# payakorn/InteriorPointMethod

Hardware: AMD Instinct MI355X
Metric: IPM iterations/sec (m=4096,n=8192 dense LP) (higher is better)
Workload: dtype f64; 1 GPU; dense synthetic LP m=4096 n=8192 fp64, seed 0, start x=s=1 y=0 (BASELINE.json configs[1]); replicas per GPU

## Files before the change

interiorpointmethod_amd/csrc/host_factor_solve.h:

```cpp
#pragma once
static inline bool sp_on(const ipm_handle* h) { return h->spf && !h->spf_off; }
static inline bool sp_level(const ipm_handle* h) {
    if (h->sp_serial || h->sp_level_mode < 0) return false;
    if (h->sp_level_mode > 0 || (h->opt.flags & IPM_FLAG_NO_DEVICE_POLLING)) return true;
    return !alone_on_device(h);
}
static inline unsigned sp_launch_grid(ipm_handle* h) {
    if (h->sp_serial) { ++h->sp_serial_launches; return 1u; }
    return (unsigned)h->sp_grid;
}
template <class Launch>
static void sp_walk(ipm_handle* h, bool by_level, bool leaves_first, Launch launch) {
    if (!by_level) { launch(sp_launch_grid(h), h->spF.rec, 0); return; }
    const size_t nlev = h->sp_lvlptr.empty() ? 0 : h->sp_lvlptr.size() - 1;
    for (size_t i = 0; i < nlev; ++i) {
        const size_t l = leaves_first ? i : nlev - 1 - i;
        const int cnt = h->sp_lvlptr[l + 1] - h->sp_lvlptr[l];
        launch((unsigned)std::min(cnt, h->sp_grid), h->sp_rec_level + h->sp_lvlptr[l], cnt);
    }
}

static int ensure_dense_B(ipm_handle* h) {
    if (h->B && h->invD) return IPM_OK;
    if (!h->no_dense) return fail(h, IPM_ERR_STATE, "handle has no dense normal-matrix buffer");
// ... 238 lines not shown
    a.L = h->B; a.ld = h->mp; a.inv = h->invD; a.done = &h->sc->done;
    a.r = r; a.z = z; a.j0 = 0;
    for (int k = k0; k < h->nblk; ++k) {
        a.k = k;
        const int nb = h->use_env ? h->env_last[k] - k + 1 : h->nblk - k;
        launch_twin<LS_TRSV_FWD>(h, (unsigned)nb, a);
    }
    a.r = z; a.z = out;
    for (int k = h->nblk - 1; k >= k0; --k) {
        a.k = k;
        a.j0 = h->use_env ? h->env_first[k] : 0;
        launch_twin<LS_TRSV_BWD>(h, (unsigned)(k - a.j0 + 1), a);
    }
}

static int enqueue_potrs_grouped(ipm_handle* h, double* r, double* out, hipEvent_t wait_last = nullptr) {
    const int GS = h->gsz;
    const int GR = GS * 128;
    const int nG = h->nblk / GS;
    const int* done = &h->sc->done;
    double* z = h->t2;
    for (int g = 0; g < nG; ++g) {
        if (wait_last && g == nG - 1) HIP_TRY(h, hipStreamWaitEvent(h->stream, wait_last, 0));
        launch_dense_gemv_n(h, h->gX + (int64_t)g * GR * GR, GR, GR, GR, r + (int64_t)g * GR, 1.0, 0.0, nullptr, z + (int64_t)g * GR);
        int below = (int)(h->mp - (int64_t)(g + 1) * GR);
        if (h->use_env) below = std::min(below, (int)((int64_t)(h->env_last[(g + 1) * GS - 1] + 1) * NB - (int64_t)(g + 1) * GR));
        if (below > 0) {
            double* rb = r + (int64_t)(g + 1) * GR;
            launch_dense_gemv_n(h, h->B + (int64_t)(g + 1) * GR * h->mp + (int64_t)g * GR, h->mp, below, GR, z + (int64_t)g * GR, -1.0, 1.0,
                                rb, rb);
        }
    }
    enqueue_block_steps(h, nG * GS, r, z, out);
    for (int g = nG - 1; g >= 0; --g) {
        launch_dense_gemv_n(h, h->gXT + (int64_t)g * GR * GR, GR, GR, GR, z + (int64_t)g * GR, 1.0, 0.0, nullptr, out + (int64_t)g * GR);
        int left = g * GR;
        const int c0 = h->use_env ? std::min(left, h->env_first[g * GS] * NB) : 0;
        left -= c0;
        if (left > 0) {
            const unsigned gx = (unsigned)((left + 511) / 512);
            launch_twin<LS_GEMV_T>(h, gx * 16u, {h->B + (int64_t)g * GR * h->mp + c0, h->mp, GR / 16, left, out + (int64_t)g * GR, h->gPart, done, gx});
            launch_twin<LS_SUB_PARTIALS>(h, (unsigned)((left + 255) / 256), {z + c0, h->gPart, left, 16, done});
        }
    }
    HIP_TRY(h, hipGetLastError());
    return IPM_OK;
}

static int enqueue_potrs(ipm_handle* h, double* r, double* out, hipEvent_t wait_last = nullptr) {
    if (sp_on(h)) {
        const int rm = std::max(16, h->sp_rmax);
        unsigned ep = ++h->sp_epoch;
        const bool fwd_done = h->sp_fwd_fused != nullptr && h->sp_fwd_fused == r;
        h->sp_fwd_fused = nullptr;
        const bool by_level = sp_level(h);
        if (!fwd_done) sp_walk(h, by_level, true, [&](unsigned grid, const SpRec* recs, int count) {
            hipLaunchKernelGGL((sp_fwd_kernel<SPC_THREADS, false>), dim3(grid), dim3(SPC_THREADS), h->sp_lds_solve, h->stream, h->spF, ep, r, h->t2, rm, recs, count);
        });
        if (!by_level) ep = ++h->sp_epoch;
        sp_walk(h, by_level, false, [&](unsigned grid, const SpRec* recs, int count) {
            hipLaunchKernelGGL((sp_bwd_kernel<SPC_THREADS, false>), dim3(grid), dim3(SPC_THREADS), 0, h->stream, h->spF, ep, h->t2, out, recs, count);
        });
        HIP_TRY(h, hipGetLastError());
        return IPM_OK;
    }
    if (h->grouped_trsv) return enqueue_potrs_grouped(h, r, out, wait_last);
    if (wait_last) HIP_TRY(h, hipStreamWaitEvent(h->stream, wait_last, 0));
    enqueue_block_steps(h, 0, r, h->t2, out);
    HIP_TRY(h, hipGetLastError());
    return IPM_OK;
}
```

interiorpointmethod_amd/csrc/host_fused.h:

```cpp
#pragma once
static bool ff_ok(const ipm_handle* h) {
    if (!h->ff_enabled || h->sparse || !polls_device(h)) return false;
    if (h->nblk < h->ff_min_nblk || h->nblk > std::min(h->ff_max_nblk, FF_MAX_NBLK) || h->np % FF_PBK) return false;
    return h->ff_forced || h->np <= 6 * h->mp;
}

static int ff_build(ipm_handle* h) {
    if (h->ff_built) return IPM_OK;
    {
        hipDeviceProp_t prop;
        HIP_TRY(h, hipGetDeviceProperties(&prop, h->device));
        if (!h->ff_forced && (strncmp(prop.gcnArchName, "gfx950", 6) != 0 || prop.multiProcessorCount != 256))
            return fail(h, IPM_ERR_STATE, "fused factor: built for a 256-CU gfx950 device (this one: %s, %d CUs)", prop.gcnArchName, prop.multiProcessorCount);
    }
    if (h->ff_workers <= 0) {
        hipDeviceProp_t prop;
        HIP_TRY(h, hipGetDeviceProperties(&prop, h->device));
        h->ff_workers = std::max(8, prop.multiProcessorCount - 1 - FF_CRIT_WGS);
    }
    const int nstages = (int)(h->np / FF_PBK);
    const int Q = std::max(1, std::min(h->ff_q, nstages));
    h->ff_q = Q;
    FFModel M;
    M.nstages = nstages;
// ... 20 lines not shown
        for (int i = 0; i < h->nblk; ++i)
            for (int c = 0; c <= i; ++c) {
                const size_t t = (size_t)ff_tile(i, c);
                if (fcnt[t] != h->ff_sched.tile_q[t] || base[t] != 1 || applied[t] != ff_limit(i, c) || paneled[t] != (ff_needs_panel(i, c) ? 1 : 0))
                    return fail(h, IPM_ERR_INVALID_ARG, "fused factor: internal error (tile %d,%d incomplete in the work list)", i, c);
            }
    }
    const size_t nit = h->ff_sched.items.size();
    HIP_TRY(h, dev_malloc(h->device, h->stream, (void**)&h->d_ff_items, sizeof(FFItem) * nit));
    HIP_TRY(h, hipMemcpyAsync(h->d_ff_items, h->ff_sched.items.data(), sizeof(FFItem) * nit, hipMemcpyHostToDevice, h->stream));
    HIP_TRY(h, dev_malloc(h->device, h->stream, (void**)&h->d_ff_tile_items, sizeof(int) * 2 * ntile));
    HIP_TRY(h, hipMemcpyAsync(h->d_ff_tile_items, h->ff_sched.tile_items.data(), sizeof(int) * ntile, hipMemcpyHostToDevice, h->stream));
    HIP_TRY(h, hipMemcpyAsync(h->d_ff_tile_items + ntile, h->ff_sched.tile_q.data(), sizeof(int) * ntile, hipMemcpyHostToDevice, h->stream));
    h->ff_flag_words = 32 + 2 * ntile + 3 * (size_t)h->nblk;
    HIP_TRY(h, dev_malloc(h->device, h->stream, (void**)&h->d_ff_flags, sizeof(unsigned) * 2 * h->ff_flag_words));
    HIP_TRY(h, dev_malloc(h->device, h->stream, (void**)&h->ff_slab, sizeof(double) * ntile * (size_t)h->ff_qmax * 128 * 128));
    if (getenv("IPM_FF_PROF")) {
        HIP_TRY(h, dev_malloc(h->device, h->stream, (void**)&h->ff_prof, sizeof(long long) * 16 * ((size_t)h->ff_workers + 1)));
        HIP_TRY(h, hipMemsetAsync(h->ff_prof, 0, sizeof(long long) * 16 * ((size_t)h->ff_workers + 1), h->stream));
    }
    if (getenv("IPM_FF_TRACE_ITEMS")) {
        const size_t words = 4 * nit + 12 * (size_t)h->nblk;
        HIP_TRY(h, dev_malloc(h->device, h->stream, (void**)&h->ff_trace, sizeof(long long) * words));
        HIP_TRY(h, hipMemsetAsync(h->ff_trace, 0, sizeof(long long) * words, h->stream));
    }
    HIP_TRY(h, hipStreamSynchronize(h->stream));
    h->ff_built = true;
    return IPM_OK;
}

static void ff_release(ipm_handle* h) {
    for (void** p : {(void**)&h->d_ff_items, (void**)&h->d_ff_flags, (void**)&h->ff_slab, (void**)&h->ff_prof, (void**)&h->ff_trace,
                     (void**)&h->d_ff_tile_items}) { dev_free(h->device, h->stream, *p); *p = nullptr; }
    h->ff_built = false;
}
static bool ff_use(ipm_handle* h) {
    if (!ff_ok(h)) return false;
    if (h->ff_built) return true;
    if (ff_build(h) == IPM_OK) return true;
    ff_release(h);
    h->ff_enabled = 0;
    (void)hipGetLastError();
    return false;
}

static int enqueue_form_factor(ipm_handle* h, hipEvent_t* ev, int mid_step, int ginv_step) {
    if (!h->ff_built) return fail(h, IPM_ERR_STATE, "fused factor: schedule not built");
    const int nblk = h->nblk;
    const size_t ntile = (size_t)nblk * (nblk + 1) / 2;
    const int* done = factor_done(h);
    hipStream_t sw = h->stream;
    unsigned* F = h->d_ff_flags;
    unsigned *ticket = F, *dbg = F + 24, *fcount = F + 32, *tprog = fcount + ntile, *lfinal = tprog + ntile, *dready = lfinal + nblk,
             *potrfdone = dready + nblk;
    unsigned* timeout = timeout_word(h);
    h->ff_potrfdone = potrfdone;
    HIP_TRY(h, hipMemsetAsync(F, 0, sizeof(unsigned) * h->ff_flag_words, sw));
    HIP_TRY(h, hipEventRecord(h->ev_fork, sw));
    long long* ctrace = h->ff_trace ? h->ff_trace + 4 * h->ff_sched.items.size() : nullptr;
    FFRoles roles;
    memset(&roles, 0, sizeof roles);
    FFChain& c = roles.chain;
    c.B = h->B; c.ldb = h->mp; c.invD = h->invD;
    c.maxbits = (const unsigned long long*)(F + 8); c.dcount = F + 10; c.maxdiag_out = &h->sc->maxdiag;
    c.dready = dready; c.potrfdone = potrfdone; c.timeout = timeout; c.dbg = dbg; c.trace = ctrace;
    c.eps = h->opt.pivot_guard_eps; c.big = h->opt.pivot_guard_big; c.shift_rel = h->shift_rel;
    c.fixed = &h->sc->fixed; c.done = done; c.nblk = nblk; c.m = (int)h->m;
    FFCrit& cc = roles.crit;
    cc.B = h->B; cc.ldb = h->mp; cc.invD = h->invD; cc.tprog = tprog; cc.tile_items = h->d_ff_tile_items;
    cc.potrfdone = potrfdone; cc.lfinal = lfinal; cc.dready = dready; cc.timeout = timeout; cc.dbg = dbg; cc.trace = ctrace;
    cc.done = done; cc.nblk = nblk;
    roles.role = F + 3;
    FFArgs a;
    memset(&a, 0, sizeof a);
    a.A = h->A; a.lda = h->np; a.d = h->d; a.B = h->B; a.ldb = h->mp; a.invD = h->invD; a.slab = h->ff_slab;
    a.items = h->d_ff_items; a.nitems = (int)h->ff_sched.items.size();
    a.ticket = ticket; a.fcount = fcount; a.tprog = tprog; a.lfinal = lfinal; a.dready = dready; a.potrfdone = potrfdone;
    a.timeout = timeout; a.dbg = dbg; a.done = done;
    { static const bool dbg_on = getenv("IPM_FF_DEBUG") != nullptr; a.dbg_words = dbg_on ? (unsigned)h->ff_flag_words : 0u; }
    a.trace = h->ff_trace;
    a.prof = h->ff_prof;
    a.tile_q = h->d_ff_tile_items + ntile;
    a.maxbits = (unsigned long long*)(F + 8); a.dcount = F + 10;
    a.nblk = nblk; a.Q = h->ff_qmax; a.nstages = (int)(h->np / FF_PBK); a.m = (int)h->m;
    if (ev) HIP_TRY(h, hipEventRecord(ev[1], sw));
    {
        const dim3 grid((unsigned)h->ff_workers + 1u + (unsigned)FF_CRIT_WGS);
        const bool instr = a.prof || a.trace;
        if (h->ff_ref_engine) {
            if (instr) hipLaunchKernelGGL((form_factor_roles_kernel<true>), grid, dim3(FF_THREADS), 0, sw, a, roles);
// ... 113 lines not shown
```

interiorpointmethod_amd/csrc/host_handle.h:

```cpp
#pragma once
static thread_local char g_err[512] = "";

static const int MAX_DEVICES = 64;
static std::atomic<int> g_live[MAX_DEVICES];
static std::atomic<bool> g_attr_set[MAX_DEVICES];

struct ipm_handle {
    int device = 0;
    hipStream_t stream = nullptr;
    bool own_stream = false;
    hipStream_t stream2 = nullptr;
    hipStream_t stream3 = nullptr;
    hipEvent_t ev_mid = nullptr, ev_res = nullptr, ev_grp = nullptr, ev_last = nullptr;
    std::vector<hipEvent_t> ev_crit, ev_bulk;
    hipEvent_t ev_fork = nullptr;
    int lookahead = 1;
    int grouped_trsv = 1;
    int gsz = 0;
    double *gXT = nullptr, *gX = nullptr, *gS = nullptr, *gPart = nullptr;
    unsigned* d_bulk_done = nullptr;
    bool no_dense = false;
    double* B_own = nullptr; double* invD_own = nullptr;
    int group_steps = 0;
    int two_level = 1;
// ... 65 lines not shown
    std::vector<int> env_last, env_first;
    bool use_env = false;
    int envelope = 1;
    bool sparse = false;
    int64_t nnz_cap = 0, nnz = 0;
    int* d_tile_order = nullptr;
    int *d_rowptr = nullptr, *d_colind = nullptr, *d_colptr = nullptr, *d_rowind = nullptr;
    double *d_rval = nullptr, *d_cval = nullptr;
    long long* stamp_buf = nullptr;
    unsigned* ff_potrfdone = nullptr;
    Scalars* sc = nullptr;
    IterRec* hist = nullptr;
    double* snap = nullptr;
    bool bnd = false;
    int bnd_nU = 0;
    double* bnd_mem = nullptr;
    bool detect = false;
    double det_eps_p = 1e-8, det_eps_d = 1e-8;
    double* det = nullptr;
    double* cert_mem = nullptr;
    int* fixed = nullptr;
    Scalars* h_sc = nullptr;
    bool haveA = false, haveBC = false, haveState = false, predictor_valid = false;
    bool fresh_state = true;
    int profiling = 0;
    double phase_ms[4] = {0, 0, 0, 0};
    hipEvent_t ev0 = nullptr, ev1 = nullptr;
    std::vector<struct LsLaunch>* ls_rec = nullptr;
    bool ls_cut = false;
    int lockstep = 0;
    unsigned spin_limit = 1u << 22;
    bool ragged_groups = true;
    bool ls_block_steps = false, potrf_stamps = false, ff_chain_mode0 = false;
    char err[512] = "";
};
struct LsLaunch { int type; LsRec rec; };
template <LsType T> static void record_twin(ipm_handle* h, unsigned gridx, const LsArgs<T>& a, unsigned lds = 0) {
    LsLaunch L{};
    L.type = T; L.rec.gridx = gridx; L.rec.lds = lds;
    memcpy(L.rec.args, &a, sizeof a);
    h->ls_rec->push_back(L);
}
template <LsType T> static void launch_twin(ipm_handle* h, unsigned grid, const LsArgs<T>& a, hipStream_t st = nullptr, unsigned lds = 0) {
    if (h->ls_rec) record_twin<T>(h, grid, a, lds);
    else LsTwin<T>::single(a, grid, lds, st ? st : h->stream);
}
template <class... P, class... Q> static void launch_untwinned(ipm_handle* h, void (*kernel)(P...), dim3 grid, dim3 block, hipStream_t st, const Q&... args) {
    if (h->ls_rec) h->ls_cut = true;
    else hipLaunchKernelGGL(kernel, grid, block, 0, st ? st : h->stream, args...);
}

static int vfail(char* err, int code, const char* fmt, va_list ap) {
    char buf[512];
    vsnprintf(buf, sizeof buf, fmt, ap);
    snprintf(g_err, sizeof g_err, "%s", buf);
    if (err) snprintf(err, 512, "%s", buf);
    return code;
}
static int fail(ipm_handle* h, int code, const char* fmt, ...) { va_list ap; va_start(ap, fmt); code = vfail(h ? h->err : nullptr, code, fmt, ap); va_end(ap); return code; }

#define HIP_TRY(h, call)                                                                      \
    do {                                                                                      \
        hipError_t e_ = (call);                                                               \
        if (e_ != hipSuccess)                                                                 \
            return fail((h), IPM_ERR_HIP, "%s failed: %s (%s:%d)", #call, hipGetErrorString(e_), \
                        __FILE__, __LINE__);                                                  \
    } while (0)

static inline int64_t round_up(int64_t v, int64_t q) { return (v + q - 1) / q * q; }

static inline int live_on_device(const ipm_handle* h) { return h->device < MAX_DEVICES ? g_live[h->device].load(std::memory_order_acquire) : 1; }
static inline bool alone_on_device(const ipm_handle* h) { return live_on_device(h) <= 1; }
static inline bool lookahead_on(const ipm_handle* h) { return h->lookahead != 0 && h->nblk > 2 && h->stream2 != nullptr; }
static inline bool wants_polling(const ipm_handle* h) { return lookahead_on(h) && h->flag_sync != 0; }
static inline bool polls_device(const ipm_handle* h) { return wants_polling(h) && alone_on_device(h); }
static inline unsigned* timeout_word(const ipm_handle* h) { return h->d_flags + 2 * (size_t)h->nblk; }
static inline const int* factor_done(const ipm_handle* h) { return h->fdone ? h->fdone : &h->sc->done; }

static std::atomic<int> g_pool_state[64];
static hipMemPool_t g_pool[64];
static std::mutex g_pool_mutex;
static bool async_alloc_ok(int device) {
    if (device < 0 || device >= 64) return false;
    int st = g_pool_state[device].load(std::memory_order_acquire);
    if (st == 0) {
        std::lock_guard<std::mutex> lock(g_pool_mutex);
        st = g_pool_state[device].load(std::memory_order_acquire);
        if (st != 0) return st == 1;
        int supported = 0;
        if (hipDeviceGetAttribute(&supported, hipDeviceAttributeMemoryPoolsSupported, device) == hipSuccess && supported) {
            hipMemPoolProps props;
            memset(&props, 0, sizeof props);
            props.allocType = hipMemAllocationTypePinned;
            props.handleTypes = hipMemHandleTypeNone;
            props.location.type = hipMemLocationTypeDevice;
            props.location.id = device;
            hipMemPool_t pool = nullptr;
            if (hipMemPoolCreate(&pool, &props) == hipSuccess && pool) {
                uint64_t keep = (uint64_t)2 << 30;
                (void)hipMemPoolSetAttribute(pool, hipMemPoolAttrReleaseThreshold, &keep);
                g_pool[device] = pool;
                st = 1;
            }
        }
        if (st == 0) st = 2;
        g_pool_state[device].store(st, std::memory_order_release);
    }
    return st == 1;
}
// ... 111 lines not shown
```

interiorpointmethod_amd/csrc/host_iteration.h:

```cpp
#pragma once
static int enqueue_solve_direction(ipm_handle* h, hipEvent_t* ev, double* dy, int corr, hipEvent_t wait_last = nullptr) {
    if (ev) HIP_TRY(h, hipEventRecord(ev[0], h->stream));
    int rc = enqueue_potrs(h, h->t1, dy, wait_last);
    if (rc) return rc;
    if (ev) HIP_TRY(h, hipEventRecord(ev[1], h->stream));
    launch_gemv_t(h, dy);
    launch_direction(h, corr);
    HIP_TRY(h, hipGetLastError());
    return IPM_OK;
}
static int enqueue_predictor(ipm_handle* h, hipEvent_t* ev, bool have_rhs = false, hipEvent_t wait_last = nullptr) {
    if (!have_rhs) launch_gemv_n(h, h->v, -1.0, -1.0, h->rb, h->t1);
    return enqueue_solve_direction(h, ev, h->dya, 0, wait_last);
}
static int enqueue_corrector(ipm_handle* h, hipEvent_t* ev) {
    launch_mu_aff(h);
    launch_corrector_rhs(h);
    launch_gemv_n(h, h->v, -1.0, -1.0, h->rb, h->t1);
    return enqueue_solve_direction(h, ev, h->dy, 1);
}

static const int EV_PER_IT = 9;

static int enqueue_iteration(ipm_handle* h, hipEvent_t* ev) {
    int rc;
    const bool all = ev && h->profiling >= 2;
    if (overlap_residuals(h)) {
        launch_scaling(h);
        const bool fused = ff_use(h);
        if (ev && !fused) HIP_TRY(h, hipEventRecord(ev[1], h->stream));
        struct Latch { ipm_handle* h; ~Latch() { h->fdone = nullptr; } } latch{h};
        h->fdone = &h->sc->done_f;
        h->ff_last = false;
        if (!fused) {
            if ((rc = enqueue_form(h, h->d))) return rc;
            if (ev) HIP_TRY(h, hipEventRecord(ev[2], h->stream));
        }
        const int rstep = h->nblk * 13 / 16;
        const int nG = h->grouped_trsv ? h->nblk / h->gsz : 0;
        const int gstep = (nG >= 2 && (nG - 1) * h->gsz - 1 < rstep) ? (nG - 1) * h->gsz - 1 : -1;
        if (fused) { if ((rc = enqueue_form_factor(h, ev, rstep, gstep))) return rc; }
        else if ((rc = enqueue_factor(h, true, rstep, gstep))) return rc;
        h->fdone = nullptr;
        if (gstep >= 0) {
            if (h->ff_last && h->ff_potrfdone) {
                hipLaunchKernelGGL(ff_gate_kernel, dim3(1), dim3(64), 0, h->stream3, h->ff_potrfdone + (h->nblk - 1), 1u, timeout_word(h), &h->sc->done);
            } else {
                HIP_TRY(h, hipEventRecord(h->ev_grp, h->stream));
                HIP_TRY(h, hipStreamWaitEvent(h->stream3, h->ev_grp, 0));
            }
            if ((rc = enqueue_group_inverses(h, nG - 1, nG, h->stream3))) return rc;
            HIP_TRY(h, hipEventRecord(h->ev_last, h->stream3));
            HIP_TRY(h, hipStreamWaitEvent(h->stream, h->ev_res, 0));
            if ((rc = enqueue_predictor(h, nullptr, true, h->ev_last))) return rc;
        } else {
            if ((rc = enqueue_group_inverses(h, 0, nG, nullptr))) return rc;
            HIP_TRY(h, hipStreamWaitEvent(h->stream, h->ev_res, 0));
            if ((rc = enqueue_predictor(h, nullptr, true))) return rc;
        }
        if ((rc = enqueue_corrector(h, nullptr))) return rc;
        launch_update(h);
        HIP_TRY(h, hipGetLastError());
        return IPM_OK;
    }
    if (all) HIP_TRY(h, hipEventRecord(ev[0], h->stream));
    if ((rc = enqueue_residuals(h))) return rc;
    h->ff_last = false;
    bool have_rhs = false;
    if (h->profiling < 2 && ff_use(h)) {
        if ((rc = enqueue_form_factor(h, ev, -1, -1))) return rc;
    } else {
        if (ev) HIP_TRY(h, hipEventRecord(ev[1], h->stream));
        if ((rc = enqueue_form(h, h->d))) return rc;
        if (ev) HIP_TRY(h, hipEventRecord(ev[2], h->stream));
        if (sp_on(h) && h->sp_fuse_fwd) {
            launch_gemv_n(h, h->v, -1.0, -1.0, h->rb, h->t1);
            have_rhs = true;
            if ((rc = enqueue_factor(h, true, -1, -1, h->t1))) return rc;
        } else if ((rc = enqueue_factor(h, true))) return rc;
    }
    if ((rc = enqueue_group_inverses(h))) return rc;
    if (all) HIP_TRY(h, hipEventRecord(ev[3], h->stream));
    if ((rc = enqueue_predictor(h, all ? ev + 4 : nullptr, have_rhs))) return rc;
    if ((rc = enqueue_corrector(h, all ? ev + 6 : nullptr))) return rc;
    launch_update(h);
    HIP_TRY(h, hipGetLastError());
    if (all) HIP_TRY(h, hipEventRecord(ev[8], h->stream));
    return IPM_OK;
}

static int read_scalars(ipm_handle* h, bool* timed_out = nullptr) {
    unsigned tmo = 0;
    unsigned* word = timeout_word(h);
    HIP_TRY(h, hipMemcpyAsync(h->h_sc, h->sc, sizeof(Scalars), hipMemcpyDeviceToHost, h->stream));
// ... 9 lines not shown
    return IPM_OK;
}

static void poll_fallback(ipm_handle* h) {
    if (h->spf) h->sp_serial = true;
    if (h->ff_last) h->ff_enabled = 0;
    else h->flag_sync = 0;
    ++h->timeouts_recovered;
}

__global__ __launch_bounds__(256) void snapshot_kernel(double* x, double* y, double* s, Scalars* sc, double* snap, int np,
                                                       int mp, int restore) {
    const int gid = blockIdx.x * 256 + threadIdx.x, gsz = gridDim.x * 256;
    double *sx = snap, *ss = snap + np, *sy = snap + 2 * (size_t)np;
    Scalars* ssc = (Scalars*)(snap + 2 * (size_t)np + mp);
    if (restore) {
        for (int j = gid; j < np; j += gsz) { x[j] = sx[j]; s[j] = ss[j]; }
        for (int i = gid; i < mp; i += gsz) y[i] = sy[i];
        if (gid == 0) *sc = *ssc;
    } else {
        for (int j = gid; j < np; j += gsz) { sx[j] = x[j]; ss[j] = s[j]; }
        for (int i = gid; i < mp; i += gsz) sy[i] = y[i];
        if (gid == 0) *ssc = *sc;
    }
}
__global__ __launch_bounds__(256) void snapshot_bounds_kernel(double* w, double* z, double* sw, double* sz, int np, int restore) {
    const int gid = blockIdx.x * 256 + threadIdx.x, gsz = gridDim.x * 256;
    for (int j = gid; j < np; j += gsz) {
        if (restore) { w[j] = sw[j]; z[j] = sz[j]; }
        else { sw[j] = w[j]; sz[j] = z[j]; }
    }
}
static int enqueue_snapshot(ipm_handle* h, int restore, hipStream_t st = nullptr) {
    const int64_t mx = h->np > h->mp ? h->np : h->mp;
    const unsigned grid = (unsigned)std::min<int64_t>((mx + 255) / 256, 256);
    hipLaunchKernelGGL(snapshot_kernel, dim3(grid), dim3(256), 0, st ? st : h->stream, h->x, h->y, h->s, h->sc, h->snap, (int)h->np,
                       (int)h->mp, restore);
    if (h->bnd) {
        const BndArgs b = bnd_args(h);
        double* sw = h->bnd_mem + 8 * (size_t)h->np;
        hipLaunchKernelGGL(snapshot_bounds_kernel, dim3(grid), dim3(256), 0, st ? st : h->stream, b.w, b.z, sw, sw + h->np, (int)h->np, restore);
    }
    HIP_TRY(h, hipGetLastError());
    return IPM_OK;
}
static bool may_poll(const ipm_handle* h) { return (h->spf && !h->sp_serial && !sp_level(h)) || wants_polling(h); }

static void fill_stats(ipm_handle* h, ipm_stats* st, double ms) {
    if (!st) return;
    const Scalars& s = *h->h_sc;
    memset(st, 0, sizeof *st);
    st->status = s.status; st->iterations = s.k; st->pivots_fixed = s.fixed; st->auto_regularized = h->auto_reg;
    st->objective_last_finite = s.obj_last_finite;
    st->objective = s.obj; st->rp_norm = s.rb_norm; st->rd_norm = s.rc_norm; st->gap = s.gap;
    st->b_norm = s.b_norm; st->c_norm = s.c_norm; st->mu = s.mu; st->mu_aff = s.mu_aff; st->sigma = s.sigma;
    st->alpha_aff_p = s.alpha_aff_p; st->alpha_aff_d = s.alpha_aff_d; st->alpha_p = s.alpha_p; st->alpha_d = s.alpha_d;
    st->solve_ms = ms;
}

static int check_ready(ipm_handle* h, const char* who) {
    if (!h) return fail(h, IPM_ERR_INVALID_ARG, "%s: NULL handle", who);
    if (!h->haveA || !h->haveBC || !h->haveState) return fail(h, IPM_ERR_STATE, "%s: A, (b,c) and a state must be set first", who);
    return IPM_OK;
}

extern "C" int ipm_newton_direction(ipm_handle* h, int corrector, double* dx, double* dy, double* ds, ipm_stats* stats) {
// ... 29 lines not shown
    if (corrector && (rc = read_scalars(h))) return rc;
    HIP_TRY(h, hipStreamSynchronize(h->stream));
    fill_stats(h, stats, 0.0);
    return IPM_OK;
}

static SmallLP small_args(ipm_handle* h, int max_steps, int auto_reg) {
    SmallLP a;
    a.A = sparse_view(h); a.m = (int)h->m; a.n = (int)h->n; a.nt = (int)((h->m + 15) / 16);
    a.bptr = h->sm_bptr; a.bi = h->sm_bi; a.bk = h->sm_bk; a.bcol = h->sm_bcol; a.bcoef = h->sm_bcoef; a.nb = h->sm_nb;
    a.x = h->x; a.y = h->y; a.s = h->s; a.b = h->b; a.c = h->c;
    a.rc = h->rc; a.d = h->d; a.v = h->v; a.q = h->q; a.dxa = h->dxa; a.dsa = h->dsa; a.dx = h->dx; a.ds = h->ds;
    a.sc = h->sc; a.hist = h->hist;
    a.eps = h->opt.pivot_guard_eps; a.big = h->opt.pivot_guard_big; a.shift_rel = h->shift_rel;
    a.max_steps = max_steps; a.auto_reg = auto_reg;
    return a;
}

static int enqueue_small(ipm_handle* h, int max_steps, int auto_reg) {
    const SmallLP a = small_args(h, max_steps, auto_reg);
    if (h->bnd && h->detect) hipLaunchKernelGGL(small_lp_bounded_detect_kernel, dim3(1), dim3(PD_THREADS), 0, h->stream, a, bnd_args(h), det_args(h));
    else if (h->bnd) hipLaunchKernelGGL(small_lp_bounded_kernel, dim3(1), dim3(PD_THREADS), 0, h->stream, a, bnd_args(h));
    else if (h->detect) hipLaunchKernelGGL(small_lp_detect_kernel, dim3(1), dim3(PD_THREADS), 0, h->stream, a, det_args(h));
    else hipLaunchKernelGGL(small_lp_kernel, dim3(1), dim3(PD_THREADS), 0, h->stream, a);
    HIP_TRY(h, hipGetLastError());
    return IPM_OK;
}

extern "C" int ipm_iterate(ipm_handle* h, int32_t n_steps, ipm_stats* stats) {
    int rc = check_ready(h, "ipm_iterate");
    if (rc) return rc;
    if (n_steps < 0) return fail(h, IPM_ERR_INVALID_ARG, "n_steps < 0");
    HIP_TRY(h, hipSetDevice(h->device));
    h->predictor_valid = false;
    std::vector<hipEvent_t> evs;
    struct EvGuard {
        std::vector<hipEvent_t>& v;
        ~EvGuard() { for (auto& e : v) if (e) (void)hipEventDestroy(e); }
    } guard{evs};
    if (h->profiling) {
        evs.assign((size_t)EV_PER_IT * n_steps, nullptr);
        for (auto& e : evs) HIP_TRY(h, hipEventCreate(&e));
    }
    float ms = 0.f;
    const int reset_k = h->fresh_state ? 1 : 0;
    h->fresh_state = false;
    if (h->small && !h->profiling) {
        hipLaunchKernelGGL(set_params_kernel, dim3(1), dim3(1), 0, h->stream, h->sc, 1e-8, 1e-8, 1e-8, h->opt.eta, 1 << 30, 1, reset_k);
        HIP_TRY(h, hipEventRecord(h->ev0, h->stream));
        if ((rc = enqueue_small(h, n_steps, 0))) return rc;
        HIP_TRY(h, hipEventRecord(h->ev1, h->stream));
        if ((rc = read_scalars(h))) return rc;
        HIP_TRY(h, hipEventElapsedTime(&ms, h->ev0, h->ev1));
        fill_stats(h, stats, ms);
        return IPM_OK;
    }
    for (int attempt = 0;; ++attempt) {
        hipLaunchKernelGGL(set_params_kernel, dim3(1), dim3(1), 0, h->stream, h->sc, 1e-8, 1e-8, 1e-8, h->opt.eta, 1 << 30, 1,
                           attempt == 0 ? reset_k : 0);
        const bool guard_poll = may_poll(h) && n_steps > 0;
        if (guard_poll && (rc = enqueue_snapshot(h, 0))) return rc;
        HIP_TRY(h, hipEventRecord(h->ev0, h->stream));
        for (int it = 0; it < n_steps; ++it)
            if ((rc = enqueue_iteration(h, h->profiling ? &evs[(size_t)it * EV_PER_IT] : nullptr))) return rc;
        if ((rc = enqueue_residuals(h))) return rc;
        HIP_TRY(h, hipEventRecord(h->ev1, h->stream));
        bool tmo = false;
        if ((rc = read_scalars(h, &tmo))) return rc;
        if (!tmo) break;
        if (attempt >= 2 || !guard_poll) return fail(h, IPM_ERR_HIP, "hand-off time-out persists with stream events");
        poll_fallback(h);
        if ((rc = enqueue_snapshot(h, 1))) return rc;
    }
    HIP_TRY(h, hipEventElapsedTime(&ms, h->ev0, h->ev1));
    if (h->profiling && n_steps > 0) {
        double ph[4] = {0, 0, 0, 0};
        for (int it = 0; it < n_steps; ++it) {
            hipEvent_t* e = &evs[(size_t)it * EV_PER_IT];
            float f = 0.f, total = 0.f;
            (void)hipEventElapsedTime(&f, e[1], e[2]); ph[0] += f;
            if (h->profiling < 2) continue;
            (void)hipEventElapsedTime(&f, e[2], e[3]); ph[1] += f;
            float s1 = 0.f, s2 = 0.f;
            (void)hipEventElapsedTime(&s1, e[4], e[5]); (void)hipEventElapsedTime(&s2, e[6], e[7]); ph[2] += s1 + s2;
            (void)hipEventElapsedTime(&total, e[0], e[8]);
            float f12 = 0.f, f23 = 0.f;
            (void)hipEventElapsedTime(&f12, e[1], e[2]); (void)hipEventElapsedTime(&f23, e[2], e[3]);
            ph[3] += total - f12 - f23 - s1 - s2;
        }
        for (int i = 0; i < 4; ++i) h->phase_ms[i] = ph[i] / n_steps;
    }
    fill_stats(h, stats, ms);
    return IPM_OK;
}

extern "C" int ipm_solve(ipm_handle* h, double tol_p, double tol_d, double tol_gap, int32_t max_iter, ipm_stats* stats) {
    int rc = check_ready(h, "ipm_solve");
    if (rc) return rc;
    if (max_iter < 0) return fail(h, IPM_ERR_INVALID_ARG, "max_iter < 0");
    HIP_TRY(h, hipSetDevice(h->device));
    h->predictor_valid = false; h->fresh_state = false;
    if (h->auto_reg) { h->auto_reg = 0; h->shift_rel = h->opt.regularize; }
    hipLaunchKernelGGL(set_params_kernel, dim3(1), dim3(1), 0, h->stream, h->sc, tol_p, tol_d, tol_gap, h->opt.eta, max_iter, 0, 1);
    HIP_TRY(h, hipEventRecord(h->ev0, h->stream));
    const int chunk = h->opt.check_every;
    const bool may_auto = h->opt.regularize == 0.0 && !(h->opt.flags & IPM_FLAG_NO_AUTO_REGULARIZE);
    if (h->small) {
        if ((rc = enqueue_small(h, 1 << 30, may_auto ? 1 : 0))) return rc;
        if ((rc = read_scalars(h))) return rc;
        if (h->h_sc->status == IPM_STATUS_NEEDS_SHIFT) {
            h->shift_rel = 1e-14; h->auto_reg = 1;
            hipLaunchKernelGGL(set_params_kernel, dim3(1), dim3(1), 0, h->stream, h->sc, tol_p, tol_d, tol_gap, h->opt.eta, max_iter, 0, 1);
            if ((rc = enqueue_small(h, 1 << 30, 0))) return rc;
            if ((rc = read_scalars(h))) return rc;
        }
        HIP_TRY(h, hipEventRecord(h->ev1, h->stream));
        HIP_TRY(h, hipEventSynchronize(h->ev1));
        float ms_ = 0.f;
        HIP_TRY(h, hipEventElapsedTime(&ms_, h->ev0, h->ev1));
        fill_stats(h, stats, ms_);
        return IPM_OK;
    }
    bool first = true;
    int recovered = 0;
    for (;;) {
        const bool snap = first || may_poll(h);
        if (snap && (rc = enqueue_snapshot(h, 0))) return rc;
        for (int i = 0; i < chunk; ++i)
            if ((rc = enqueue_iteration(h, nullptr))) return rc;
        bool tmo = false;
        if ((rc = read_scalars(h, &tmo))) return rc;
        if (tmo) {
            if (!snap || ++recovered > 2) return fail(h, IPM_ERR_HIP, "hand-off time-out persists with stream events");
            poll_fallback(h);
// ... 20 lines not shown
```

interiorpointmethod_amd/csrc/host_residuals.h:

```cpp
#pragma once
static void launch_gemv_n(ipm_handle* h, const double* v, double sa, double sb, const double* add, double* out,
                          hipStream_t st = nullptr) {
    if (h->sparse) launch_twin<LS_SPMV_CSR>(h, (unsigned)((h->mp + 15) / 16), {sparse_view(h), (int)h->mp, v, sa, sb, add, out, &h->sc->done}, st);
    else launch_untwinned(h, gemv_n_kernel, dim3((unsigned)(h->mp / 4)), dim3(256), st, h->A, h->np, (int)h->mp, (int)h->np, v, sa, sb, add, out, &h->sc->done);
}
static void launch_gemv_t(ipm_handle* h, const double* u, hipStream_t st = nullptr) {
    if (h->sparse) launch_twin<LS_SPMV_CSC_T>(h, (unsigned)((h->np + 15) / 16), {sparse_view(h), (int)h->np, u, h->atp, &h->sc->done}, st);
    else launch_untwinned(h, gemv_t_kernel, dim3((unsigned)((h->np + 511) / 512), (unsigned)h->rc_chunks), dim3(256), st, h->A, h->np, h->rows_per_chunk, (int)h->np, u, h->atp, &h->sc->done);
}

template <LsType T> static void launch_vec_step(ipm_handle* h, void (*bounded)(VecArgs, BndArgs), hipStream_t st = nullptr) {
    if (h->bnd) launch_untwinned(h, bounded, dim3(h->vblk), dim3(VBLK), st, vec_args(h), bnd_args(h));
    else launch_twin<T>(h, (unsigned)h->vblk, {vec_args(h), 0}, st);
}
static void launch_prepare(ipm_handle* h, hipStream_t st) {
    if (h->bnd && h->detect) launch_untwinned(h, prepare_bounded_detect_kernel, dim3(h->vblk), dim3(VBLK), st, vec_args(h), bnd_args(h));
    else if (h->detect) launch_twin<LS_PREPARE_DETECT>(h, (unsigned)h->vblk, {vec_args(h), det_args(h)}, st);
    else launch_vec_step<LS_PREPARE>(h, prepare_bounded_kernel, st);
}
static void launch_stop_test(ipm_handle* h, hipStream_t st) {
    if (h->bnd && h->detect) launch_untwinned(h, stop_test_bounded_detect_kernel, dim3(1), dim3(64), st, vec_args(h), bnd_args(h), det_args(h));
    else if (h->bnd) launch_untwinned(h, stop_test_bounded_kernel, dim3(1), dim3(64), st, vec_args(h), bnd_args(h));
    else if (h->detect) launch_twin<LS_STOP_TEST_DETECT>(h, 1u, {vec_args(h), det_args(h)}, st);
    else launch_twin<LS_STOP_TEST>(h, 1u, {vec_args(h), 0}, st);
}
static void launch_scaling(ipm_handle* h) {
    if (h->bnd) hipLaunchKernelGGL(scaling_bounded_kernel, dim3(h->vblk), dim3(VBLK), 0, h->stream, vec_args(h), bnd_args(h));
    else hipLaunchKernelGGL(scaling_kernel, dim3(h->vblk), dim3(VBLK), 0, h->stream, vec_args(h));
}
static void launch_direction(ipm_handle* h, int corr) {
    if (h->bnd) launch_untwinned(h, direction_bounded_kernel, dim3(h->vblk), dim3(VBLK), nullptr, vec_args(h), corr, bnd_args(h));
    else launch_twin<LS_DIRECTION>(h, (unsigned)h->vblk, {vec_args(h), corr});
}
static void launch_mu_aff(ipm_handle* h) { launch_vec_step<LS_MU_AFF>(h, mu_aff_bounded_kernel); }
static void launch_corrector_rhs(ipm_handle* h) { launch_vec_step<LS_CORR_RHS>(h, corrector_rhs_bounded_kernel); }
static void launch_update(ipm_handle* h) { launch_vec_step<LS_UPDATE>(h, update_bounded_kernel); }

static int enqueue_residuals(ipm_handle* h, hipStream_t st = nullptr) {
    launch_gemv_n(h, h->x, 1.0, -1.0, h->b, h->rb, st);
    launch_gemv_t(h, h->y, st);
    launch_prepare(h, st);
    launch_stop_test(h, st);
    HIP_TRY(h, hipGetLastError());
    return IPM_OK;
}

static int enqueue_residual_stream(ipm_handle* h, hipStream_t chain) {
    HIP_TRY(h, hipEventRecord(h->ev_mid, chain));
    HIP_TRY(h, hipStreamWaitEvent(h->stream3, h->ev_mid, 0));
    int rc = enqueue_residuals(h, h->stream3);
    if (rc) return rc;
    launch_gemv_n(h, h->v, -1.0, -1.0, h->rb, h->t1, h->stream3);
    HIP_TRY(h, hipEventRecord(h->ev_res, h->stream3));
    HIP_TRY(h, hipGetLastError());
    return IPM_OK;
}
static bool overlap_residuals(const ipm_handle* h) {
    return h->stream3 != nullptr && h->profiling < 2;
}
```

interiorpointmethod_amd/csrc/ipm_api.hip:

```cpp
#include <hip/hip_runtime.h>
#include <hip/hip_ext.h>
#include <math.h>
#include <stdarg.h>
#include <stdio.h>
#include <stdlib.h>
#include <string.h>

#include <deque>
#include <vector>

#include "../../include/ipm_hip.h"
#include "gemm_nt_f64.h"
#include "adat_syrk_f64.h"
#include "chol_update_f64.h"
#include "potrf_f64.h"
#include "sparse_ops.h"
#include "trsv_grouped.h"
#include "getrf_f64.h"
#include "small_lp.h"
#include "sparse_chol.h"
#include "sparse_symbolic.h"
#include "vector_ops.h"
#include "form_factor.h"
#include "lockstep.h"
// ... 47 lines not shown
}

extern "C" int ipm_workspace_bytes_csc(int64_t m, int64_t n, int64_t nnz, size_t* bytes) {
    if (!bytes || m <= 0 || n <= 0 || nnz <= 0) return fail(nullptr, IPM_ERR_INVALID_ARG, "bad arguments to ipm_workspace_bytes_csc");
    *bytes = make_layout(m, n, nnz).total;
    return IPM_OK;
}

extern "C" int ipm_workspace_bytes_opts(int64_t m, int64_t n, const ipm_options* opts, size_t* bytes) {
    if (!bytes || m <= 0 || n <= 0) return fail(nullptr, IPM_ERR_INVALID_ARG, "bad arguments to ipm_workspace_bytes_opts");
    const int64_t nnz = opts && opts->sparse_nnz > 0 ? opts->sparse_nnz : 0;
    *bytes = make_layout(m, n, nnz, layout_no_dense(m, nnz, opts ? opts->flags : 0u)).total;
    return IPM_OK;
}

static void read_env_switches(ipm_handle* h) {
    if (const char* e = getenv("IPM_TEST_SPIN_LIMIT")) h->spin_limit = (unsigned)std::max(1, atoi(e));
    if (const char* e = getenv("IPM_ENVELOPE")) h->envelope = atoi(e);
    if (const char* e = getenv("IPM_LOOKAHEAD")) h->lookahead = atoi(e);
    if (const char* e = getenv("IPM_GROUPED_TRSV")) h->grouped_trsv = atoi(e);
    if (getenv("IPM_LS_BLOCK_STEPS")) h->ls_block_steps = true;
    if (const char* e = getenv("IPM_RAGGED_GROUPS")) h->ragged_groups = atoi(e) != 0;
    if (const char* e = getenv("IPM_FLAG_SYNC")) h->flag_sync = atoi(e);
    if (const char* e = getenv("IPM_BULK_VARIANT")) h->bulk_variant = atoi(e);
    if (const char* e = getenv("IPM_TWO_LEVEL")) h->two_level = atoi(e);
    if (const char* e = getenv("IPM_GROUP_STEPS")) h->group_steps = atoi(e);
    if (const char* e = getenv("IPM_FUSED_SMALL")) h->fused_small = atoi(e);
    if (const char* e = getenv("IPM_LIST_FORM")) h->list_form_opt = atoi(e);
    if (getenv("IPM_POTRF_STAMPS")) h->potrf_stamps = true;
    if (const char* e = getenv("IPM_FUSED_FACTOR")) { if (!strcmp(e, "force")) { h->ff_enabled = 1; h->ff_min_nblk = 3; h->ff_forced = true; } else h->ff_enabled = atoi(e); }
    if (const char* e = getenv("IPM_FF_MAX_NBLK")) h->ff_max_nblk = atoi(e);
    if (const char* e = getenv("IPM_FF_CHAIN_MODE")) h->ff_chain_mode0 = atoi(e) == 0;
    if (const char* e = getenv("IPM_FF_REF_ENGINE")) h->ff_ref_engine = atoi(e) != 0;
    if (const char* e = getenv("IPM_FF_Q")) h->ff_q = std::max(1, std::min(16, atoi(e)));
}

extern "C" int ipm_create(int device, int64_t m, int64_t n, const ipm_options* opts, void* workspace,
                          size_t workspace_bytes, void* stream, ipm_handle** out) {
    if (!out) return fail(nullptr, IPM_ERR_INVALID_ARG, "out is NULL");
    *out = nullptr;
    if (m <= 0 || n <= 0 || m > (1 << 20) || n > (1 << 24)) return fail(nullptr, IPM_ERR_INVALID_ARG, "bad problem size %lld x %lld", (long long)m, (long long)n);
    int ndev = 0;
    if (hipGetDeviceCount(&ndev) != hipSuccess || ndev <= 0) return fail(nullptr, IPM_ERR_NO_DEVICE, "no HIP device visible");
    if (device < 0 || device >= ndev) return fail(nullptr, IPM_ERR_INVALID_ARG, "device %d out of range (%d visible)", device, ndev);
    ipm_handle* h = new ipm_handle();
    h->device = device;
    if (opts) h->opt = *opts; else ipm_default_options(&h->opt);
    if (h->opt.check_every < 1) h->opt.check_every = 1;
    if (!(h->opt.eta > 0.0)) h->opt.eta = 0.91;
    if (!(h->opt.pivot_guard_big > 0.0)) h->opt.pivot_guard_big = 1e64;
    if (!(h->opt.regularize >= 0.0)) h->opt.regularize = 0.0;
    h->shift_rel = h->opt.regularize;
    read_env_switches(h);
    if (h->opt.sparse_nnz < 0) h->opt.sparse_nnz = 0;
    h->sparse = h->opt.sparse_nnz > 0;
    h->nnz_cap = h->opt.sparse_nnz;
    h->no_dense = layout_no_dense(m, h->opt.sparse_nnz, h->opt.flags);
    Layout L = make_layout(m, n, h->opt.sparse_nnz, h->no_dense);
    h->m = m; h->n = n; h->mp = L.mp; h->np = L.np; h->nblk = L.nblk;
    h->rc_chunks = L.rc_chunks; h->rows_per_chunk = L.rows_per_chunk; h->vblk = L.vblk;
    h->ws_bytes = L.total;
#define CREATE_TRY(call)                                                                       \
    do {                                                                                       \
        hipError_t e_ = (call);                                                                \
        if (e_ != hipSuccess) {                                                                \
            int rc_ = fail(nullptr, IPM_ERR_HIP, "%s failed: %s", #call, hipGetErrorString(e_)); \
// ... 487 lines not shown
```

interiorpointmethod_amd/csrc/trsv_grouped.h:

```cpp
#pragma once
#include <hip/hip_runtime.h>
#include <stdint.h>
#include "gemm_nt_f64.h"

namespace ipm {

constexpr int GS_MAX = 8;

__device__ __forceinline__ void group_diag_transpose_kernel_body(const double* __restrict__ invD, double* XT, double* X, int b0, int GS, const int* done,
                                                                  const unsigned bx_, const unsigned by_, const unsigned bz_) {
    if (done && *done) return;
    __shared__ double tile[32][33];
    const int64_t GR = (int64_t)GS * 128;
    const int b = b0 + bz_, g = b / GS, a = b % GS;
    const double* src = invD + (int64_t)b * 128 * 128;
    double* dst = XT + (int64_t)g * GR * GR + (int64_t)(a * 128) * GR + a * 128;
    double* dsx = X + (int64_t)g * GR * GR + (int64_t)(a * 128) * GR + a * 128;
    const int bx = bx_ * 32, by = by_ * 32;
    for (int j = threadIdx.y; j < 32; j += 8) {
        double v = src[(int64_t)(by + j) * 128 + bx + threadIdx.x];
        tile[j][threadIdx.x] = v;
        dsx[(int64_t)(by + j) * GR + bx + threadIdx.x] = v;
    }
    __syncthreads();
    for (int j = threadIdx.y; j < 32; j += 8) dst[(int64_t)(bx + j) * GR + by + threadIdx.x] = tile[threadIdx.x][j];
}
__global__ void group_diag_transpose_kernel(const double* __restrict__ invD, double* XT, double* X, int b0, int GS, const int* done) {
    group_diag_transpose_kernel_body(invD, XT, X, b0, GS, done, blockIdx.x, blockIdx.y, blockIdx.z);
}

__device__ __forceinline__ void sub_partials_kernel_body(double* z, const double* __restrict__ part, int np, int rc,
                                                           const int* done, const unsigned bx_, const unsigned gx_) {
    if (done && *done) return;
    const int c = bx_ * 256 + threadIdx.x;
    if (c >= np) return;
    double s = 0.0;
    int r = 0;
    for (; r + 8 <= rc; r += 8) {
        double t[8];
#pragma unroll
        for (int q = 0; q < 8; ++q) t[q] = part[(int64_t)(r + q) * np + c];
#pragma unroll
        for (int q = 0; q < 8; ++q) s += t[q];
    }
    for (; r < rc; ++r) s += part[(int64_t)r * np + c];
    z[c] -= s;
}
__global__ __launch_bounds__(256) void sub_partials_kernel(double* z, const double* __restrict__ part, int np, int rc,
                                                           const int* done) { sub_partials_kernel_body(z, part, np, rc, done, blockIdx.x, gridDim.x); }

}
```

interiorpointmethod_amd/csrc/vector_ops.h:

```cpp
#pragma once
#include <hip/hip_runtime.h>
#include <stdint.h>
#include "gemm_nt_f64.h"

namespace ipm {

constexpr int VBLK = 256;
constexpr int MAXPART = 64;

struct Scalars {
    double b_norm, c_norm;
    double rb_norm, rc_norm, gap, obj;
    double mu, mu_aff, sigma;
    double alpha_aff_p, alpha_aff_d, alpha_p, alpha_d;
    double maxdiag;
    double e1, e2, e3, eta;
    double obj_last_finite;
    int done, status, k, max_iter, fixed, force, fixed_first;
    int done_f;
};

struct IterRec {
    int k, fixed;
    double obj, rb, rc, gap, mu, sigma, aap, aad, ap, ad;
// ... 365 lines not shown
__global__ __launch_bounds__(VBLK) void corrector_rhs_kernel(VecArgs a) { corrector_rhs_kernel_body(a, blockIdx.x, gridDim.x); }
__global__ __launch_bounds__(VBLK) void corrector_rhs_bounded_kernel(VecArgs a, BndArgs bd) { corrector_rhs_kernel_body<true>(a, blockIdx.x, gridDim.x, bd); }

template <bool Bounded = false>
__device__ __forceinline__ void update_kernel_body(VecArgs a, const unsigned bx_, const unsigned gx_, BndArgs bd = BndArgs{}) {
    if (a.sc->done) return;
    const int gid = bx_ * VBLK + threadIdx.x, gsz = gx_ * VBLK;
    const double eta = a.sc->eta;
    const double ap = fmin(1.0, eta * min_partials(a.part, P_MINP, a.nblk));
    const double ad = fmin(1.0, eta * min_partials(a.part, P_MIND, a.nblk));
    for (int j = gid; j < a.n; j += gsz) {
        a.x[j] += ap * a.dx[j];
        a.s[j] += ad * a.ds[j];
        if constexpr (Bounded) {
            bd.w[j] += ap * bd.dw[j];
            bd.z[j] += ad * bd.dz[j];
        }
    }
    for (int i = gid; i < a.m; i += gsz) a.y[i] += ad * a.dy[i];
    if (gid == 0) {
        Scalars* sc = a.sc;
        const int k = sc->k;
        if (k == 0) sc->fixed_first = sc->fixed;
        IterRec r;
        r.k = k; r.fixed = sc->fixed; r.obj = sc->obj; r.rb = sc->rb_norm; r.rc = sc->rc_norm; r.gap = sc->gap;
        r.mu = sc->mu; r.sigma = sc->sigma; r.aap = sc->alpha_aff_p; r.aad = sc->alpha_aff_d; r.ap = ap; r.ad = ad;
        a.hist[k % HIST_CAP] = r;
        sc->alpha_p = ap; sc->alpha_d = ad; sc->k = k + 1;
    }
}
__global__ __launch_bounds__(VBLK) void update_kernel(VecArgs a) { update_kernel_body(a, blockIdx.x, gridDim.x); }
__global__ __launch_bounds__(VBLK) void update_bounded_kernel(VecArgs a, BndArgs bd) { update_kernel_body<true>(a, blockIdx.x, gridDim.x, bd); }

__global__ void fill_kernel(double* out, int n, double value) {
    int i = blockIdx.x * blockDim.x + threadIdx.x;
    if (i < n) out[i] = value;
}

__global__ __launch_bounds__(VBLK) void norm2_kernel(const double* v, int n, double* out) {
    __shared__ double red[VBLK];
    double acc = 0.0;
    for (int i = threadIdx.x; i < n; i += VBLK) acc += v[i] * v[i];
    acc = block_sum(acc, red);
    if (threadIdx.x == 0) *out = sqrt(acc);
}

__global__ __launch_bounds__(VBLK) void bnd_norm2_kernel(const double* b, int m, const double* u, int n, double* out) {
    __shared__ double red[VBLK];
    double acc = 0.0;
    for (int i = threadIdx.x; i < m; i += VBLK) acc += b[i] * b[i];
    for (int j = threadIdx.x; j < n; j += VBLK) { const double uj = u[j]; if (bnd_in(uj)) acc += uj * uj; }
    acc = block_sum(acc, red);
    if (threadIdx.x == 0) *out = sqrt(acc);
}

__global__ void bnd_fill_kernel(const double* u, double* w, double* z, int n, double value, int mask_only) {
    const int j = blockIdx.x * blockDim.x + threadIdx.x;
    if (j >= n) return;
    if (!bnd_in(u[j])) { w[j] = 0.0; z[j] = 0.0; }
    else if (!mask_only) { w[j] = value; z[j] = value; }
}

}
```

Baseline: 266.9 iterations/s.

## Fold update with next-iteration scaling, flag zeroing, and sub-partials into gemv

Fuses the end-of-iteration update kernel with the next iteration's scaling computation and the zeroing of the fused-factor flag words, so one launch and one memset drop out of each iteration. In the grouped backward triangular solve, the partial-sum subtraction is folded into the following group's diagonal gemv kernel, removing one launch per group. The price is extra state tracking (next_ready, ff_zeroed) to skip scaling and memset safely. There is also a correctness risk: the fused scaling runs inside the same grid as the update without a grid-wide barrier, so it may read x and s values that other blocks have not yet written.

```diff
diff --git a/interiorpointmethod_amd/csrc/host_factor_solve.h b/interiorpointmethod_amd/csrc/host_factor_solve.h
--- a/interiorpointmethod_amd/csrc/host_factor_solve.h
+++ b/interiorpointmethod_amd/csrc/host_factor_solve.h
@@ -294,15 +294,19 @@
         }
     }
     enqueue_block_steps(h, nG * GS, r, z, out);
+    const bool fold = fold_on(h) && !h->use_env && GR % 256 == 0;
     for (int g = nG - 1; g >= 0; --g) {
-        launch_dense_gemv_n(h, h->gXT + (int64_t)g * GR * GR, GR, GR, GR, z + (int64_t)g * GR, 1.0, 0.0, nullptr, out + (int64_t)g * GR);
+        if (fold && g < nG - 1)
+            hipLaunchKernelGGL(gemv_n_sub_partials_kernel, dim3((unsigned)(64 + g)), dim3((unsigned)GR), 0, h->stream, h->gXT + (int64_t)g * GR * GR,
+                               GR, z, h->gPart, (g + 1) * GR, 16, out + (int64_t)g * GR, done);
+        else launch_dense_gemv_n(h, h->gXT + (int64_t)g * GR * GR, GR, GR, GR, z + (int64_t)g * GR, 1.0, 0.0, nullptr, out + (int64_t)g * GR);
         int left = g * GR;
         const int c0 = h->use_env ? std::min(left, h->env_first[g * GS] * NB) : 0;
         left -= c0;
         if (left > 0) {
             const unsigned gx = (unsigned)((left + 511) / 512);
             launch_twin<LS_GEMV_T>(h, gx * 16u, {h->B + (int64_t)g * GR * h->mp + c0, h->mp, GR / 16, left, out + (int64_t)g * GR, h->gPart, done, gx});
-            launch_twin<LS_SUB_PARTIALS>(h, (unsigned)((left + 255) / 256), {z + c0, h->gPart, left, 16, done});
+            if (!fold) launch_twin<LS_SUB_PARTIALS>(h, (unsigned)((left + 255) / 256), {z + c0, h->gPart, left, 16, done});
         }
     }
     HIP_TRY(h, hipGetLastError());
diff --git a/interiorpointmethod_amd/csrc/host_fused.h b/interiorpointmethod_amd/csrc/host_fused.h
--- a/interiorpointmethod_amd/csrc/host_fused.h
+++ b/interiorpointmethod_amd/csrc/host_fused.h
@@ -76,7 +76,7 @@
 static void ff_release(ipm_handle* h) {
     for (void** p : {(void**)&h->d_ff_items, (void**)&h->d_ff_flags, (void**)&h->ff_slab, (void**)&h->ff_prof, (void**)&h->ff_trace,
                      (void**)&h->d_ff_tile_items}) { dev_free(h->device, h->stream, *p); *p = nullptr; }
-    h->ff_built = false;
+    h->ff_built = false; h->ff_zeroed = false;
 }
 static bool ff_use(ipm_handle* h) {
     if (!ff_ok(h)) return false;
@@ -99,7 +99,8 @@
              *potrfdone = dready + nblk;
     unsigned* timeout = timeout_word(h);
     h->ff_potrfdone = potrfdone;
-    HIP_TRY(h, hipMemsetAsync(F, 0, sizeof(unsigned) * h->ff_flag_words, sw));
+    if (!h->ff_zeroed) HIP_TRY(h, hipMemsetAsync(F, 0, sizeof(unsigned) * h->ff_flag_words, sw));
+    h->ff_zeroed = false;
     HIP_TRY(h, hipEventRecord(h->ev_fork, sw));
     long long* ctrace = h->ff_trace ? h->ff_trace + 4 * h->ff_sched.items.size() : nullptr;
     FFRoles roles;
diff --git a/interiorpointmethod_amd/csrc/host_handle.h b/interiorpointmethod_amd/csrc/host_handle.h
--- a/interiorpointmethod_amd/csrc/host_handle.h
+++ b/interiorpointmethod_amd/csrc/host_handle.h
@@ -121,6 +121,9 @@
     unsigned spin_limit = 1u << 22;
     bool ragged_groups = true;
     bool ls_block_steps = false, potrf_stamps = false, ff_chain_mode0 = false;
+    int fold_launches = 1;
+    bool next_ready = false;
+    bool ff_zeroed = false;
     char err[512] = "";
 };
 struct LsLaunch { int type; LsRec rec; };
@@ -164,6 +167,7 @@
 static inline bool wants_polling(const ipm_handle* h) { return lookahead_on(h) && h->flag_sync != 0; }
 static inline bool polls_device(const ipm_handle* h) { return wants_polling(h) && alone_on_device(h); }
 static inline unsigned* timeout_word(const ipm_handle* h) { return h->d_flags + 2 * (size_t)h->nblk; }
+static inline bool fold_on(const ipm_handle* h) { return h->fold_launches != 0 && !h->sparse && !h->ls_rec; }
 static inline const int* factor_done(const ipm_handle* h) { return h->fdone ? h->fdone : &h->sc->done; }
 
 static std::atomic<int> g_pool_state[64];
diff --git a/interiorpointmethod_amd/csrc/host_iteration.h b/interiorpointmethod_amd/csrc/host_iteration.h
--- a/interiorpointmethod_amd/csrc/host_iteration.h
+++ b/interiorpointmethod_amd/csrc/host_iteration.h
@@ -25,8 +25,10 @@
 static int enqueue_iteration(ipm_handle* h, hipEvent_t* ev) {
     int rc;
     const bool all = ev && h->profiling >= 2;
+    const bool d_ready = h->next_ready;
+    h->next_ready = false;
     if (overlap_residuals(h)) {
-        launch_scaling(h);
+        if (!d_ready) launch_scaling(h);
         const bool fused = ff_use(h);
         if (ev && !fused) HIP_TRY(h, hipEventRecord(ev[1], h->stream));
         struct Latch { ipm_handle* h; ~Latch() { h->fdone = nullptr; } } latch{h};
@@ -59,7 +61,8 @@
             if ((rc = enqueue_predictor(h, nullptr, true))) return rc;
         }
         if ((rc = enqueue_corrector(h, nullptr))) return rc;
-        launch_update(h);
+        if (fold_on(h)) launch_update_scaling(h);
+        else launch_update(h);
         HIP_TRY(h, hipGetLastError());
         return IPM_OK;
     }
@@ -135,6 +138,7 @@
     }
 }
 static int enqueue_snapshot(ipm_handle* h, int restore, hipStream_t st = nullptr) {
+    if (restore) h->next_ready = false;
     const int64_t mx = h->np > h->mp ? h->np : h->mp;
     const unsigned grid = (unsigned)std::min<int64_t>((mx + 255) / 256, 256);
     hipLaunchKernelGGL(snapshot_kernel, dim3(grid), dim3(256), 0, st ? st : h->stream, h->x, h->y, h->s, h->sc, h->snap, (int)h->np,
@@ -230,7 +234,7 @@
     if (rc) return rc;
     if (n_steps < 0) return fail(h, IPM_ERR_INVALID_ARG, "n_steps < 0");
     HIP_TRY(h, hipSetDevice(h->device));
-    h->predictor_valid = false;
+    h->predictor_valid = false; h->next_ready = false;
     std::vector<hipEvent_t> evs;
     struct EvGuard {
         std::vector<hipEvent_t>& v;
@@ -297,7 +301,7 @@
     if (rc) return rc;
     if (max_iter < 0) return fail(h, IPM_ERR_INVALID_ARG, "max_iter < 0");
     HIP_TRY(h, hipSetDevice(h->device));
-    h->predictor_valid = false; h->fresh_state = false;
+    h->predictor_valid = false; h->fresh_state = false; h->next_ready = false;
     if (h->auto_reg) { h->auto_reg = 0; h->shift_rel = h->opt.regularize; }
     hipLaunchKernelGGL(set_params_kernel, dim3(1), dim3(1), 0, h->stream, h->sc, tol_p, tol_d, tol_gap, h->opt.eta, max_iter, 0, 1);
     HIP_TRY(h, hipEventRecord(h->ev0, h->stream));
diff --git a/interiorpointmethod_amd/csrc/host_residuals.h b/interiorpointmethod_amd/csrc/host_residuals.h
--- a/interiorpointmethod_amd/csrc/host_residuals.h
+++ b/interiorpointmethod_amd/csrc/host_residuals.h
@@ -35,6 +35,14 @@
 static void launch_mu_aff(ipm_handle* h) { launch_vec_step<LS_MU_AFF>(h, mu_aff_bounded_kernel); }
 static void launch_corrector_rhs(ipm_handle* h) { launch_vec_step<LS_CORR_RHS>(h, corrector_rhs_bounded_kernel); }
 static void launch_update(ipm_handle* h) { launch_vec_step<LS_UPDATE>(h, update_bounded_kernel); }
+static void launch_update_scaling(ipm_handle* h) {
+    static const bool keep_words = getenv("IPM_FF_DEBUG") != nullptr;
+    unsigned* zero = (h->ff_built && !keep_words) ? h->d_ff_flags : nullptr;
+    if (h->bnd) hipLaunchKernelGGL(update_scaling_bounded_kernel, dim3(h->vblk), dim3(VBLK), 0, h->stream, vec_args(h), bnd_args(h), zero, (int)h->ff_flag_words);
+    else hipLaunchKernelGGL(update_scaling_kernel, dim3(h->vblk), dim3(VBLK), 0, h->stream, vec_args(h), zero, (int)h->ff_flag_words);
+    h->next_ready = true;
+    h->ff_zeroed = zero != nullptr;
+}
 
 static int enqueue_residuals(ipm_handle* h, hipStream_t st = nullptr) {
     launch_gemv_n(h, h->x, 1.0, -1.0, h->b, h->rb, st);
diff --git a/interiorpointmethod_amd/csrc/ipm_api.hip b/interiorpointmethod_amd/csrc/ipm_api.hip
--- a/interiorpointmethod_amd/csrc/ipm_api.hip
+++ b/interiorpointmethod_amd/csrc/ipm_api.hip
@@ -103,6 +103,7 @@
     if (const char* e = getenv("IPM_FF_MAX_NBLK")) h->ff_max_nblk = atoi(e);
     if (const char* e = getenv("IPM_FF_CHAIN_MODE")) h->ff_chain_mode0 = atoi(e) == 0;
     if (const char* e = getenv("IPM_FF_REF_ENGINE")) h->ff_ref_engine = atoi(e) != 0;
+    if (const char* e = getenv("IPM_FOLD_LAUNCHES")) h->fold_launches = atoi(e);
     if (const char* e = getenv("IPM_FF_Q")) h->ff_q = std::max(1, std::min(16, atoi(e)));
 }
 
diff --git a/interiorpointmethod_amd/csrc/trsv_grouped.h b/interiorpointmethod_amd/csrc/trsv_grouped.h
--- a/interiorpointmethod_amd/csrc/trsv_grouped.h
+++ b/interiorpointmethod_amd/csrc/trsv_grouped.h
@@ -2,6 +2,7 @@
 #include <hip/hip_runtime.h>
 #include <stdint.h>
 #include "gemm_nt_f64.h"
+#include "vector_ops.h"
 
 namespace ipm {
 
@@ -49,4 +50,17 @@
 __global__ __launch_bounds__(256) void sub_partials_kernel(double* z, const double* __restrict__ part, int np, int rc,
                                                            const int* done) { sub_partials_kernel_body(z, part, np, rc, done, blockIdx.x, gridDim.x); }
 
+__global__ __launch_bounds__(GS_MAX * 128) __attribute__((amdgpu_num_vgpr(26))) void gemv_n_sub_partials_kernel(const double* __restrict__ XT, int GR, double* z,
+                                                                           const double* __restrict__ part, int left, int rc,
+                                                                           double* out, const int* done) {
+    __shared__ double vl[GS_MAX * 128];
+    const unsigned q = (unsigned)GR / 256;
+    if (blockIdx.x >= 64) { sub_partials_kernel_body(z, part, left, rc, done, (blockIdx.x - 64) * q, 0); return; }
+    const int c0 = left - GR;
+    vl[threadIdx.x] = z[c0 + threadIdx.x];
+    sub_partials_kernel_body(vl, part + c0, left, rc, done, 0, 0);
+    __syncthreads();
+    gemv_n_kernel_body(XT, GR, GR, GR, vl, 1.0, 0.0, nullptr, out, done, blockIdx.x * q, 0);
 }
+
+}
diff --git a/interiorpointmethod_amd/csrc/vector_ops.h b/interiorpointmethod_amd/csrc/vector_ops.h
--- a/interiorpointmethod_amd/csrc/vector_ops.h
+++ b/interiorpointmethod_amd/csrc/vector_ops.h
@@ -421,6 +421,21 @@
 __global__ __launch_bounds__(VBLK) void update_kernel(VecArgs a) { update_kernel_body(a, blockIdx.x, gridDim.x); }
 __global__ __launch_bounds__(VBLK) void update_bounded_kernel(VecArgs a, BndArgs bd) { update_kernel_body<true>(a, blockIdx.x, gridDim.x, bd); }
 
+__device__ __forceinline__ void zero_words(unsigned* zero, int nzero) {
+    if (!zero) return;
+    for (int i = blockIdx.x * VBLK + threadIdx.x; i < nzero; i += gridDim.x * VBLK) zero[i] = 0u;
+}
+__global__ __launch_bounds__(VBLK) void update_scaling_kernel(VecArgs a, unsigned* zero, int nzero) {
+    zero_words(zero, nzero);
+    update_kernel_body(a, blockIdx.x, gridDim.x);
+    scaling_kernel_body(a);
+}
+__global__ __launch_bounds__(VBLK) void update_scaling_bounded_kernel(VecArgs a, BndArgs bd, unsigned* zero, int nzero) {
+    zero_words(zero, nzero);
+    update_kernel_body<true>(a, blockIdx.x, gridDim.x, bd);
+    scaling_kernel_body<true>(a, bd);
+}
+
 __global__ void fill_kernel(double* out, int n, double value) {
     int i = blockIdx.x * blockDim.x + threadIdx.x;
     if (i < n) out[i] = value;
```

New measurement: 268.0 iterations/s (median of 6 runs). About the same (+0.4%).
